# Keep-Passion/ImageStitch

Measured on AMD Instinct MI355X. Metric: image-pairs/sec (2048x2048 grayscale, SURF+BF), higher is better.
Workload: dtype f32

## Files before the change

imagestitch_amd/csrc/surf_kernels.hip:

```cpp
#include "common.h"
#include "detmath.h"
#include <math.h>
#include <float.h>
#include <string.h>
#include <stdlib.h>
#include <algorithm>
#include <vector>

#define GAS __attribute__((address_space(1)))
typedef GAS const uint8_t *g_cu8;
typedef GAS const int32_t *g_ci32;
typedef GAS float *g_f32;
typedef GAS const float *g_cf32;
typedef GAS int32_t *g_i32;
__device__ __forceinline__ int cv_round_f(float v) { return (int)rintf(v); }
__device__ __forceinline__ uint8_t round_u8_pos(float v) { return (uint8_t)__float_as_uint(v + 12582912.f); }
__device__ __forceinline__ int cv_round_d(double v) { return (int)rint(v); }
__device__ __forceinline__ int cv_floor_d(double v) { return (int)floor(v); }
__device__ __forceinline__ int cv_ceil_d(double v) { return (int)ceil(v); }

__device__ __forceinline__ int wave_incl_scan(int v)
{
    const int lane = threadIdx.x & 63;
#pragma unroll
// ... 655 lines not shown
        int t = base + threadIdx.x;
        if (t < n) { SortKey k = make_key(R.cand[t]); t1[threadIdx.x] = k.k1; t2[threadIdx.x] = k.k2; t3[threadIdx.x] = k.k3; }
        __syncthreads();
        const int k0 = part * 64, k1e = min(k0 + 64, n - base);
        if (idx < n) {
            bool tie = false;
#pragma unroll 8
            for (int k = k0; k < k1e; k++) {
                const unsigned long long a = t1[k];
                rank += (a > mk.k1) ? 1 : 0;
                tie |= (a == mk.k1);
            }
            if (tie)
                for (int k = k0; k < k1e; k++)
                    if (t1[k] == mk.k1) rank += (t2[k] < mk.k2 || (t2[k] == mk.k2 && t3[k] < mk.k3)) ? 1 : 0;
        }
        __syncthreads();
    }
    partial[part][lane] = rank;
    __syncthreads();
    if (part == 0 && idx < n) {
        rank = partial[0][lane] + partial[1][lane] + partial[2][lane] + partial[3][lane];
        vfsms_keypoint kp;
        kp.x = me.x; kp.y = me.y; kp.size = me.size; kp.angle = -1.f; kp.response = me.response;
        kp.octave = me.octave; kp.class_id = cand_class_id(R, pats, me);
        R.kps[rank] = kp;
    }
}

#define SORT_BUCKETS 1024
struct SortRec { unsigned long long k1, k2, k3; int idx, pad; };
__device__ __forceinline__ int sort_bucket(unsigned long long k1)
{
    const int b = (int)((uint32_t)(k1 >> 32) >> 18) - (133 << 5);
    return min(max(b, 0), SORT_BUCKETS - 1);
}
__global__ __launch_bounds__(1024) void k_bucket_sort(const RoiDev *rois)
{
    const RoiDev &R = rois[blockIdx.x];
    const int n = min(R.counters[0], R.cap);
    if (n <= 0) return;
    __shared__ int hist[SORT_BUCKETS], base[SORT_BUCKETS], cursor[SORT_BUCKETS], wsum[16];
    const int tid = threadIdx.x, lane = tid & 63, wid = tid >> 6;
    hist[tid] = 0; cursor[tid] = 0;
    __syncthreads();
    for (int i = tid; i < n; i += 1024) atomicAdd(&hist[sort_bucket(make_key(R.cand[i]).k1)], 1);
    __syncthreads();
    {
        const int rb = SORT_BUCKETS - 1 - tid;
        const int v = hist[rb];
        int incl = wave_incl_scan(v);
        if (lane == 63) wsum[wid] = incl;
        __syncthreads();
        int off = 0;
        for (int k = 0; k < wid; k++) off += wsum[k];
        base[rb] = off + incl - v;
    }
    __syncthreads();
    SortRec *S = reinterpret_cast<SortRec *>(R.patch);
    for (int i = tid; i < n; i += 1024) {
        const SortKey k = make_key(R.cand[i]);
        const int b = sort_bucket(k.k1);
        const int pos = base[b] + atomicAdd(&cursor[b], 1);
        SortRec r; r.k1 = k.k1; r.k2 = k.k2; r.k3 = k.k3; r.idx = i; r.pad = 0;
        S[pos] = r;
    }
    R.keep_pos[tid] = base[tid]; R.order[tid] = hist[tid];
}

#define BRANK_STAGE 1024
__global__ __launch_bounds__(256) void k_bucket_rank(const RoiDev *rois, const LayerPat *pats)
{
    const RoiDev &R = rois[blockIdx.y];
    const int n = min(R.counters[0], R.cap);
    const int p0 = blockIdx.x * 256;
    if (p0 >= n) return;
    const int p = p0 + (int)threadIdx.x;
    const bool live = p < n;
    const GAS unsigned long long *S = (const GAS unsigned long long *)R.patch;
    static_assert(sizeof(SortRec) == 32, "k_bucket_rank reads the records as four 64-bit words");
    g_ci32 bpos = (g_ci32)R.keep_pos, bcnt = (g_ci32)R.order;
    __shared__ unsigned long long key1[BRANK_STAGE];
    __shared__ int span[2];
    SortRec me; me.k1 = me.k2 = me.k3 = 0; me.idx = 0;
    int lo = 0, hi = 0;
    if (live) {
        me.k1 = S[4 * p]; me.k2 = S[4 * p + 1]; me.k3 = S[4 * p + 2]; me.idx = (int)(uint32_t)S[4 * p + 3];
        const int b = sort_bucket(me.k1);
        lo = bpos[b]; hi = lo + bcnt[b];
        if (threadIdx.x == 0) span[0] = lo;
        if (p == min(p0 + 255, n - 1)) span[1] = hi;
    }
    __syncthreads();
    const int s0 = span[0], s1 = span[1];
    int rank = lo;
    auto tie = [&](int q) {
        const unsigned long long a2 = S[4 * q + 1], a3 = S[4 * q + 2];
        return (a2 < me.k2 || (a2 == me.k2 && a3 < me.k3)) ? 1 : 0;
    };
    if (s1 - s0 <= BRANK_STAGE) {
        for (int q = s0 + (int)threadIdx.x; q < s1; q += 256) key1[q - s0] = S[4 * q];
        __syncthreads();
        if (live) {
            int q = lo;
            for (; q + 4 <= hi; q += 4) {
                unsigned long long a[4];
#pragma unroll
                for (int u = 0; u < 4; u++) a[u] = key1[q - s0 + u];
#pragma unroll
                for (int u = 0; u < 4; u++) {
                    rank += (a[u] > me.k1) ? 1 : 0;
                    if (a[u] == me.k1 && q + u != p) rank += tie(q + u);
                }
            }
            for (; q < hi; q++) {
                const unsigned long long a1 = key1[q - s0];
                rank += (a1 > me.k1) ? 1 : 0;
                if (a1 == me.k1 && q != p) rank += tie(q);
            }
        }
    } else if (live) {
        for (int q = lo; q < hi; q++) {
            const unsigned long long a1 = S[4 * q];
            rank += (a1 > me.k1) ? 1 : 0;
            if (a1 == me.k1 && q != p) rank += tie(q);
        }
    }
    if (!live) return;
    Cand c;
    {
        constexpr int CW = sizeof(Cand) / 4;
        g_ci32 src = (g_ci32)R.cand + (size_t)me.idx * CW;
        int32_t *cw = (int32_t *)&c;
#pragma unroll
        for (int w = 0; w < CW; w++) cw[w] = src[w];
    }
    vfsms_keypoint kp;
    kp.x = c.x; kp.y = c.y; kp.size = c.size; kp.angle = -1.f; kp.response = c.response;
    kp.octave = c.octave; kp.class_id = cand_class_id(R, pats, c);
    {
        constexpr int KW = sizeof(vfsms_keypoint) / 4;
        g_i32 dst = (g_i32)R.kps + (size_t)rank * KW;
        const int32_t *kw = (const int32_t *)&kp;
#pragma unroll
        for (int w = 0; w < KW; w++) dst[w] = kw[w];
    }
}

__device__ __forceinline__ float fast_atan2_deg(float y, float x)
{
    const float s = (float)(180 / 3.1415926535897932384626433832795);
    const float p1 = 0.9997878412794807f * s, p3 = -0.3258083974640975f * s;
    const float p5 = 0.1555786518463281f * s, p7 = -0.04432655554792128f * s;
    float ax = fabsf(x), ay = fabsf(y);
    float a, c, c2;
    if (ax >= ay) {
        c = ay / (ax + (float)DBL_EPSILON);
        c2 = c * c;
        a = (((p7 * c2 + p5) * c2 + p3) * c2 + p1) * c;
    } else {
        c = ax / (ay + (float)DBL_EPSILON);
        c2 = c * c;
        a = 90.f - (((p7 * c2 + p5) * c2 + p3) * c2 + p1) * c;
    }
    if (x < 0) a = 180.f - a;
    if (y < 0) a = 360.f - a;
    return a;
}

#ifndef ORI_KP
#define ORI_KP 2
#endif
typedef float ori_f2 __attribute__((ext_vector_type(2)));
__device__ __forceinline__ void orientation_block(const RoiDev &R, const SurfTables *T, const int k0, const int n, int upright)
{
    __shared__ __attribute__((aligned(16))) float2 XY[ORI_KP][128];
    __shared__ __attribute__((aligned(16))) uint8_t Zb[ORI_KP][9][128];
    __shared__ float mod_s[ORI_KP][72], sx_s[ORI_KP][72], sy_s[ORI_KP][72];
    __shared__ int nvalid[ORI_KP], state[ORI_KP];
    const int tid = threadIdx.x;
    const int kq = __builtin_amdgcn_readfirstlane(tid >> 7), t = tid & 127;
    if (tid < ORI_KP) { nvalid[tid] = 0; state[tid] = 0; }
    __syncthreads();
    {
        const int k = k0 + kq;
        int valid = 0;
        uint32_t m0 = 0, m1 = 0, m2 = 0;
        float2 xy = make_float2(0.f, 0.f);
        if (k < n) {
            const vfsms_keypoint kp = R.kps[k];
            const float s = kp.size * 1.2f / 9.0f;
            const int gws = 2 * cv_round_f(2 * s);
            const int srows = R.h + 1, scols = R.w + 1, sw = R.w + 1;
            if (srows < gws || scols < gws) {
                if (t == 0) { R.kps[k].size = -1.f; state[kq] = 1; }
            } else if (upright) {
                if (t == 0) { R.kps[k].angle = 270.f; state[kq] = 1; }
            } else if (t < T->nOriSamples) {
                int x = cv_round_f(kp.x + T->aptx[t] * s - (float)(gws - 1) / 2);
                int y = cv_round_f(kp.y + T->apty[t] * s - (float)(gws - 1) / 2);
                if (!(y < 0 || y >= srows - gws || x < 0 || x >= scols - gws)) {
                    const float ratio = (float)gws / 4;
                    const int r2 = cv_round_f(ratio * 2), r4 = cv_round_f(ratio * 4);
                    g_ci32 p0 = (g_ci32)R.sum + (size_t)y * sw + x;
                    g_ci32 p2 = p0 + (size_t)r2 * sw, p4 = p0 + (size_t)r4 * sw;
                    const int a00 = p0[0], a02 = p0[r2], a04 = p0[r4];
                    const int a20 = p2[0], a24 = p2[r4];
                    const int a40 = p4[0], a42 = p4[r2], a44 = p4[r4];
                    const float wA = 1.f / ((float)r2 * (float)r4);
                    float wB = wA;
                    if (r4 - r2 != r2) wB = 1.f / ((float)(r4 - r2) * (float)r4);
                    const int vx0 = a00 + a42 - a40 - a02, vx1 = a02 + a44 - a42 - a04;
                    const int vy0 = a00 + a24 - a20 - a04, vy1 = a20 + a44 - a40 - a24;
                    double dxd = 0; dxd += (double)(-((float)vx0 * wA)); dxd += (double)((float)vx1 * wB);
                    double dyd = 0; dyd += (double)((float)vy0 * wA); dyd += (double)(-((float)vy1 * wB));
                    const float vx = (float)dxd, vy = (float)dyd;
                    const float aw = T->aptw[t];
                    const float xx = vx * aw, yy = vy * aw;
                    xy = make_float2(xx, yy);
                    const int ang = cv_round_f(fast_atan2_deg(yy, xx));
                    const uint32_t *mrow = T->oriMask[min(max(ang, 0), 360)];
                    m0 = mrow[0]; m1 = mrow[1]; m2 = mrow[2];
                    valid = 1;
                }
            }
        } else if (t == 0) state[kq] = 1;
        XY[kq][t] = xy;
        Zb[kq][0][t] = (uint8_t)m0; Zb[kq][1][t] = (uint8_t)(m0 >> 8); Zb[kq][2][t] = (uint8_t)(m0 >> 16); Zb[kq][3][t] = (uint8_t)(m0 >> 24);
        Zb[kq][4][t] = (uint8_t)m1; Zb[kq][5][t] = (uint8_t)(m1 >> 8); Zb[kq][6][t] = (uint8_t)(m1 >> 16); Zb[kq][7][t] = (uint8_t)(m1 >> 24);
        Zb[kq][8][t] = (uint8_t)m2;
        const unsigned long long m = __ballot(valid);
        if ((tid & 63) == 0 && m) atomicAdd(&nvalid[kq], __popcll(m));
    }
    __syncthreads();
    if (tid < ORI_KP * 72) {
        const int q = tid / 72, w = tid - q * 72;
        if (state[q] == 0 && nvalid[q] > 0) {
            const int nori = T->nOriSamples;
            const uint8_t *zrow = Zb[q][w >> 3];
            const int bit = w & 7;
            ori_f2 acc = {0.f, 0.f};
            for (int j = 0; j < nori; j += 8) {
                const uint2 z8 = *reinterpret_cast<const uint2 *>(&zrow[j]);
                const uint32_t za = (z8.x >> bit) & 0x01010101u, zb = (z8.y >> bit) & 0x01010101u;
                const float4 p01 = *reinterpret_cast<const float4 *>(&XY[q][j]), p23 = *reinterpret_cast<const float4 *>(&XY[q][j + 2]);
                const float4 p45 = *reinterpret_cast<const float4 *>(&XY[q][j + 4]), p67 = *reinterpret_cast<const float4 *>(&XY[q][j + 6]);
#define ORI_ACC(Z, N, P, XC, YC) do { float mf; asm("v_cvt_f32_ubyte" #N " %0, %1" : "=v"(mf) : "v"(Z)); \
                                           acc = __builtin_elementwise_fma((ori_f2){P.XC, P.YC}, (ori_f2){mf, mf}, acc); } while (0)
                ORI_ACC(za, 0, p01, x, y); ORI_ACC(za, 1, p01, z, w); ORI_ACC(za, 2, p23, x, y); ORI_ACC(za, 3, p23, z, w);
                ORI_ACC(zb, 0, p45, x, y); ORI_ACC(zb, 1, p45, z, w); ORI_ACC(zb, 2, p67, x, y); ORI_ACC(zb, 3, p67, z, w);
#undef ORI_ACC
            }
            const float sumx = acc.x, sumy = acc.y;
            mod_s[q][w] = sumx * sumx + sumy * sumy;
            sx_s[q][w] = sumx; sy_s[q][w] = sumy;
        }
    }
    __syncthreads();
    {
        const int q = __builtin_amdgcn_readfirstlane(tid >> 6), lane = tid & 63;
        if (q < ORI_KP && state[q] == 0) {
            const int k = k0 + q;
            if (nvalid[q] == 0) {
                if (lane == 0) R.kps[k].size = -1.f;
            } else {
                float bm = mod_s[q][lane]; int bi = lane;
                if (!(bm > 0.f)) bm = 0.f;
                if (lane < 8) { float m2 = mod_s[q][64 + lane]; if (m2 > bm) { bm = m2; bi = 64 + lane; } }
#pragma unroll
                for (int off = 32; off >= 1; off >>= 1) {
                    const float om = __shfl_xor(bm, off, 64); const int oi = __shfl_xor(bi, off, 64);
                    if (om > bm || (om == bm && oi < bi)) { bm = om; bi = oi; }
                }
                if (lane == 0) {
                    float bestx = 0, besty = 0;
                    if (bm > 0.f) { bestx = sx_s[q][bi]; besty = sy_s[q][bi]; }
                    R.kps[k].angle = fast_atan2_deg(-besty, bestx);
                }
            }
        }
    }
}

#ifdef VFSMS_DESC_TIMING
__device__ unsigned long long g_desc_cycles[8];
#define DT_MARK(ph) do { if (threadIdx.x == 0) { unsigned long long _n = clock64(); atomicAdd(&g_desc_cycles[ph], _n - _t0); _t0 = _n; } } while (0)
#define DT_START unsigned long long _t0 = clock64()
extern "C" int vfsms_debug_desc_cycles(unsigned long long *out) { return hipMemcpyFromSymbol(out, HIP_SYMBOL(g_desc_cycles), sizeof(unsigned long long) * 8) == hipSuccess ? 0 : -3; }
__device__ unsigned long long g_desc_trips[4];
#define DT_TRIP(n) do {} while (0)
__device__ unsigned long long g_desc_unit_cycles[4];
#define DT_UNIT_BEGIN unsigned long long _u0 = clock64()
#define DT_UNIT_END(n) do { _uacc[n] += clock64() - _u0; _ucnt[n]++; } while (0)
extern "C" int vfsms_debug_desc_unit_cycles(unsigned long long *out) { return hipMemcpyFromSymbol(out, HIP_SYMBOL(g_desc_unit_cycles), sizeof(unsigned long long) * 4) == hipSuccess ? 0 : -3; }
extern "C" int vfsms_debug_desc_trips(unsigned long long *out) { return hipMemcpyFromSymbol(out, HIP_SYMBOL(g_desc_trips), sizeof(unsigned long long) * 4) == hipSuccess ? 0 : -3; }
#else
#define DT_MARK(ph) do {} while (0)
#define DT_START do {} while (0)
#define DT_TRIP(n) do {} while (0)
#define DT_UNIT_BEGIN do {} while (0)
#define DT_UNIT_END(n) do {} while (0)
#endif
#ifndef VFSMS_EXP
#define VFSMS_EXP 0
#endif
#ifndef DESC_WBUF
#define DESC_WBUF 15360
#endif
__device__ __forceinline__ void origin_chain(float *row, float s, const float d, const int n)
{
    int i = 0;
    for (; i + 4 <= n; i += 4) {
        const float a = s, b = a + d, c = b + d, e = c + d;
        s = e + d;
        row[i] = a; row[i + 1] = b; row[i + 2] = c; row[i + 3] = e;
    }
    for (; i < n; i++, s += d) row[i] = s;
}

struct WinGeom {
    int win; float sin_dir, cos_dir;
    int h, w, stride; g_cu8 img;
    g_cu8 pair;
    int upright, usx, usy;
};

__device__ __forceinline__ int win_sample_xy(const WinGeom &G, double px, double py)
{
    const int ncols1 = G.w - 1, nrows1 = G.h - 1;
    const int ix = (int)px, iy = (int)py;
    if (px >= 0.0 && py >= 0.0 && ix < ncols1 && iy < nrows1) {
        const float a = (float)__builtin_amdgcn_fract(px), b = (float)__builtin_amdgcn_fract(py);
        g_cu8 p = G.img + (size_t)iy * G.stride + ix;
        const float v = p[0] * (1.f - a) * (1.f - b) + p[1] * a * (1.f - b) + p[G.stride] * (1.f - a) * b + p[G.stride + 1] * a * b;
        return (int)(uint8_t)cv_round_f(v);
    }
    const int x = min(max(cv_round_d(px), 0), ncols1);
    const int y = min(max(cv_round_d(py), 0), nrows1);
    return (int)G.img[(size_t)y * G.stride + x];
}
__device__ __forceinline__ int win_sample_upright(const WinGeom &G, int i, int j)
{
    const int x = min(max(G.usx + i, 0), G.w - 1);
    const int y = min(max(G.usy - j, 0), G.h - 1);
    return (int)G.img[(size_t)y * G.stride + x];
}

typedef float float2v __attribute__((ext_vector_type(2)));
__device__ __forceinline__ float bilinear_pk(uint32_t top, float a, float b)
{
    const float na = 1.f - a, nb = 1.f - b;
    const float2v w = {na, a};
    const float2v r0 = {(float)(top & 0xff), (float)((top >> 16) & 0xff)};
    const float2v r1 = {(float)((top >> 8) & 0xff), (float)(top >> 24)};
    float2v p = r0 * w, q = r1 * w;
    const float2v nb2 = {nb, nb}, b2 = {b, b};
    p = p * nb2; q = q * b2;
    return ((p.x + p.y) + q.x) + q.y;
}
#ifndef STAGE_ILP
#define STAGE_ILP 4
#endif
#define UNIT_W (8 * STAGE_ILP)
#ifndef BORDER_ILP
#define BORDER_ILP 2
#endif
#ifndef STAGE_FRAC_FIRST
#define STAGE_FRAC_FIRST 1
#endif
template <int N>
__device__ __forceinline__ void stage_round(g_cu8 ubase, const uint32_t pw, const double c, const double sn, const double sxc, const double syc,
                                            const int jlane, uint8_t *wrow)
{
    uint32_t top[N];
    const double jd = (double)jlane;
    const double px0 = __builtin_fma(jd, c, sxc), py0 = __builtin_fma(jd, -sn, syc);
#if STAGE_FRAC_FIRST
    float fa[N], fb[N];
#pragma unroll
    for (int u = 0; u < N; u++) {
        const double px = u ? px0 + (double)(8 * u) * c : px0, py = u ? py0 - (double)(8 * u) * sn : py0;
        const uint32_t off = ((uint32_t)__umul24((uint32_t)(int)py, pw) + (uint32_t)(int)px) << 1;
        fa[u] = (float)__builtin_amdgcn_fract(px); fb[u] = (float)__builtin_amdgcn_fract(py);
        top[u] = *(GAS const uint32_t *)(ubase + off);
    }
#pragma unroll
    for (int u = 0; u < N; u++) wrow[8 * u] = round_u8_pos(bilinear_pk(top[u], fa[u], fb[u]));
#else
    double px[N], py[N];
    px[0] = px0; py[0] = py0;
#pragma unroll
    for (int u = 1; u < N; u++) { px[u] = px[0] + (double)(8 * u) * c; py[u] = py[0] - (double)(8 * u) * sn; }
#pragma unroll
    for (int u = 0; u < N; u++) {
        const uint32_t off = ((uint32_t)__umul24((uint32_t)(int)py[u], pw) + (uint32_t)(int)px[u]) << 1;
        top[u] = *(GAS const uint32_t *)(ubase + off);
    }
#pragma unroll
    for (int u = 0; u < N; u++) {
        const float a = (float)__builtin_amdgcn_fract(px[u]), b = (float)__builtin_amdgcn_fract(py[u]);
        wrow[8 * u] = round_u8_pos(bilinear_pk(top[u], a, b));
    }
#endif
}

template <int NW>
__device__ __forceinline__ void stage_rows(const WinGeom &G, const float *sx_row, const float *sy_row,
                                           int r0, int nrows, uint8_t *dst, uint8_t *strip_in)
{
    const int win = __builtin_amdgcn_readfirstlane(G.win);
    r0 = __builtin_amdgcn_readfirstlane(r0); nrows = __builtin_amdgcn_readfirstlane(nrows);
    const int lane = threadIdx.x & 63, wv = NW == 1 ? 0 : __builtin_amdgcn_readfirstlane((int)(threadIdx.x >> 6));
    const int li = lane >> 3, lj = lane & 7;
    const int strips = (nrows + 7) >> 3;
    const double c = (double)G.cos_dir, sn = (double)G.sin_dir;
    const int ncols1 = __builtin_amdgcn_readfirstlane(G.w) - 1, nrows1 = __builtin_amdgcn_readfirstlane(G.h) - 1;
    const uint64_t bp = (uint64_t)G.pair;
    g_cu8 ubase = (g_cu8)(((uint64_t)(uint32_t)__builtin_amdgcn_readfirstlane((uint32_t)(bp >> 32)) << 32) |
                          (uint64_t)(uint32_t)__builtin_amdgcn_readfirstlane((uint32_t)bp));
    const uint32_t pw = (uint32_t)(ncols1 + 1);
    const int gfull = win >> 3, tailc = win & 7;
    int nb = NW == 1 ? 1 : (gfull + 7) >> 3;
#if VFSMS_EXP & 16
    nb = (gfull + 3) >> 2;
#endif
    const int gbase = gfull / nb, grem = gfull - gbase * nb;
    const int total = strips * nb;
    if (!G.upright) {
        const int tid = NW == 1 ? lane : (int)threadIdx.x;
        if (tid < strips) {
            const int ia = min(r0 + tid * 8, VFSMS_MAX_WIN - 1), ib = min(min(r0 + tid * 8 + 7, r0 + nrows - 1), VFSMS_MAX_WIN - 1);
// ... 233 lines not shown
            __syncthreads();
            DT_MARK(3);
            for (int p0 = 0; p0 < cn; p0 += DESC_PASS) {
                const int pn = min(DESC_PASS, cn - p0);
                for (int e = threadIdx.x; e < pn * 21; e += 256) {
                    const int r = (int)(((uint32_t)e * 3121u) >> 16), dx = e - 21 * r;
                    if (tail_ok) {
                        const AreaRec cx = REC[dx];
                        float w[AREA_TAIL];
                        area_tail_weights(cx, nmin, w);
                        rowsum[e] = area_row_tab_w(WINBUF + (p0 + r) * win, cx, nmin, nmax, w);
                    } else
                        rowsum[e] = area_row_tab(WINBUF + (p0 + r) * win, REC[dx], nmin, nmax);
                }
                __syncthreads();
                const int s0 = c0 + p0, s1 = s0 + pn;
                for (int o = threadIdx.x; o < 441; o += 256) {
                    const int dy = (int)(((uint32_t)o * 3121u) >> 16), dx = o - 21 * dy;
                    const AreaRec ry = REC[dy];
                    const int a = max(ry.j0, s0), b = min(ry.j0 + ry.n, s1);
                    if (dy < dyA || dy >= dyB || a >= b) continue;
                    float sum = a == ry.j0 ? 0.f : acc[o];
                    for (int s = a; s < b; s++) {
                        const int t = s - ry.j0;
                        const float rb = rowsum[(s - s0) * 21 + dx];
                        if (t == 0) sum = ry.a0 * rb;
                        else sum += (t < ry.n - 1 ? ry.af : ry.al) * rb;
                    }
                    if (b == ry.j0 + ry.n) PATCH[dy][dx] = area_out(sum, mode, inv_area);
                    else acc[o] = sum;
                }
                if (p0 + DESC_PASS < cn) __syncthreads();
            }
            DT_MARK(4);
        }
    }
    __syncthreads();
    if (band >= 0) {
        if (threadIdx.x < 21) R.patch[(size_t)k * VFSMS_PATCH_ROW + band * 21 + threadIdx.x] = PATCH[band][threadIdx.x];
    } else {
        for (int o = threadIdx.x; o < 441; o += 256) R.patch[(size_t)k * VFSMS_PATCH_ROW + o] = PATCH[o / 21][o % 21];
    }
    DT_MARK(5);
}

#define DESC_NCLS 4

__device__ __forceinline__ int desc_class(float size)
{
    const float s = size * 1.2f / 9.0f;
    const int win = min((int)((20 + 1) * s), VFSMS_MAX_WIN);
    return win > 256 ? 0 : win > 128 ? 1 : win > 64 ? 2 : 3;
}

__global__ __launch_bounds__(1024) void k_desc_order(const RoiDev *rois)
{
    const RoiDev &R = rois[blockIdx.x];
    const int n = min(R.counters[0], R.cap);
    __shared__ int cnt[DESC_NCLS], base[DESC_NCLS], cur[DESC_NCLS];
    if (threadIdx.x < DESC_NCLS) { cnt[threadIdx.x] = 0; cur[threadIdx.x] = 0; }
    __syncthreads();
    const int lane = threadIdx.x & 63;
    for (int k0 = 0; k0 < n; k0 += 1024) {
        const int k = k0 + threadIdx.x;
        const float size = k < n ? R.kps[k].size : -1.f;
        const int cls = size > 0 ? desc_class(size) : -1;
#pragma unroll
        for (int c = 0; c < DESC_NCLS; c++) {
            const unsigned long long m = __ballot(cls == c);
            if (m && lane == __ffsll((long long)m) - 1) atomicAdd(&cnt[c], __popcll(m));
        }
    }
    __syncthreads();
    if (threadIdx.x == 0) {
        int acc = 0;
        for (int c = 0; c < DESC_NCLS; c++) { base[c] = acc; acc += cnt[c]; R.counters[12 + c] = cnt[c]; }
    }
    __syncthreads();
    for (int k0 = 0; k0 < n; k0 += 1024) {
        const int k = k0 + threadIdx.x;
        const float size = k < n ? R.kps[k].size : -1.f;
        const int cls = size > 0 ? desc_class(size) : -1;
#pragma unroll
        for (int c = 0; c < DESC_NCLS; c++) {
            const unsigned long long m = __ballot(cls == c);
            if (!m) continue;
            const int leader = __ffsll((long long)m) - 1;
            int start = 0;
            if (lane == leader) start = atomicAdd(&cur[c], __popcll(m));
            start = __shfl(start, leader, 64);
            if (cls == c) R.order[base[c] + start + __popcll(m & ((1ull << lane) - 1))] = k;
        }
    }
}

#define DESC_HEADS DESC_PLAN_HEADS
#define DESC_HEAD_STRIDE 64

__global__ __launch_bounds__(256) void k_desc_plan(const RoiDev *rois, int nrois, DescPlan *plan, int big_grid)
{
    __shared__ int c[VFSMS_MAX_ROIS][4];
    for (int e = threadIdx.x; e < nrois * 4; e += 256) c[e >> 2][e & 3] = rois[e >> 2].counters[12 + (e & 3)];
    __syncthreads();
    if (threadIdx.x == 0) {
        int acc = 0, total = 0;
        for (int q = 0; q < DESC_HEADS; q++) {
            plan->big_start[q] = acc;
            for (int r = q; r < nrois; r += DESC_HEADS) { plan->seg_base[r][0] = acc; acc += c[r][0]; }
            plan->big_n0[q] = acc - plan->big_start[q];
            for (int r = q; r < nrois; r += DESC_HEADS) {
                plan->seg_base[r][1] = acc; acc += c[r][1];
                plan->seg_base[r][2] = acc; acc += c[r][2];
            }
            plan->big_tickets[q] = acc - plan->big_start[q];
        }
        total = acc;
        const int split = total < big_grid * 48 ? 21 : 1;
        plan->split = split;
        for (int q = 0; q < DESC_HEADS; q++) plan->big_tickets[q] += (split - 1) * plan->big_n0[q];
        acc = 0;
        for (int q = 0; q < DESC_HEADS; q++) {
            plan->small_start[q] = acc;
            for (int r = q; r < nrois; r += DESC_HEADS) { plan->seg_base[r][3] = acc; acc += c[r][3]; }
            plan->small_tickets[q] = acc - plan->small_start[q];
        }
    }
}

__global__ __launch_bounds__(256) void k_desc_recs(const RoiDev *rois, const DescPlan *plan, DescRec *big, DescRec *small, int upright)
{
    const int roi = blockIdx.y;
    const RoiDev &R = rois[roi];
    const int p = blockIdx.x * 256 + threadIdx.x;
    const int c0 = R.counters[12], c1 = R.counters[13], c2 = R.counters[14], c3 = R.counters[15];
    if (p >= c0 + c1 + c2 + c3) return;
    const int cls = p < c0 ? 0 : p < c0 + c1 ? 1 : p < c0 + c1 + c2 ? 2 : 3;
    const int idx = p - (cls > 0 ? c0 : 0) - (cls > 1 ? c1 : 0) - (cls > 2 ? c2 : 0);
    const int k = R.order[p];
    const vfsms_keypoint kp = R.kps[k];
    DescRec rec;
    rec.roi = roi; rec.k = k; rec.pad = 0; rec.x = kp.x; rec.y = kp.y;
    rec.win = (int)((20 + 1) * (kp.size * 1.2f / 9.0f));
    rec.sin_dir = 0.f; rec.cos_dir = 0.f;
    if (!upright) {
        const float dir = kp.angle * (float)(3.1415926535897932384626433832795 / 180);
        double sd, cd;
        det_sincos((double)dir, &sd, &cd);
        rec.sin_dir = -(float)sd;
        rec.cos_dir = (float)cd;
    }
    (cls < 3 ? big : small)[plan->seg_base[roi][cls] + idx] = rec;
}

__global__ __launch_bounds__(ORI_KP * 128, 8) void k_orientation(const RoiDev *rois, const SurfTables *T, int upright)
{
    const RoiDev &R = rois[blockIdx.y];
    const int n = min(R.counters[0], R.cap);
    const int k0 = blockIdx.x * ORI_KP;
    if (k0 >= n) return;
    orientation_block(R, T, k0, n, upright);
}

#define DESC_SMALL_WIN 64
struct SmallLds { uint8_t win[DESC_SMALL_WIN * DESC_SMALL_WIN + 64]; float sx[DESC_SMALL_WIN + 8], sy[DESC_SMALL_WIN + 8]; AreaRec rec[AREA_RECS]; int rec_win; uint8_t strip_in[DESC_SMALL_WIN / 8 + 8]; };

__device__ __forceinline__ void wave_sync_lds()
{
    __builtin_amdgcn_fence(__ATOMIC_ACQ_REL, "wavefront");
    __builtin_amdgcn_wave_barrier();
}

__device__ void describe_small(const RoiDev &R, const AreaRec *area_tab, const DescRec &rec, int upright, SmallLds &L)
{
    const int lane = threadIdx.x & 63;
    const int k = rec.k;
    WinGeom G;
    G.win = min(rec.win, DESC_SMALL_WIN);
    G.h = R.h; G.w = R.w; G.stride = R.stride; G.img = (g_cu8)R.img; G.pair = (g_cu8)R.pair;
    G.upright = upright; G.usx = 0; G.usy = 0; G.sin_dir = rec.sin_dir; G.cos_dir = rec.cos_dir;
    const int win = G.win;
    const int dsz = 21;
    if (L.rec_win != win) {
        wave_sync_lds();
        const int *src = (const int *)(area_tab + (size_t)max(win, dsz) * AREA_RECS);
        for (int e = lane; e < AREA_RECS * 8; e += 64) ((int *)L.rec)[e] = src[e];
        if (lane == 0) L.rec_win = win;
    }
    if (!upright) {
        const float sin_dir = rec.sin_dir, cos_dir = rec.cos_dir;
        if (lane < 2) {
            const float win_offset = -(float)(win - 1) / 2;
            const float sx0 = rec.x + win_offset * cos_dir + win_offset * sin_dir, sy0 = rec.y - win_offset * sin_dir + win_offset * cos_dir;
            origin_chain(lane == 0 ? L.sx : L.sy, lane == 0 ? sx0 : sy0, lane == 0 ? sin_dir : cos_dir, win);
        }
    } else {
        const float win_offset = -(float)(win - 1) / 2;
        G.usx = cv_round_f(rec.x + win_offset);
        G.usy = cv_round_f(rec.y - win_offset);
    }
    wave_sync_lds();
    stage_rows<1>(G, L.sx, L.sy, 0, win, L.win, L.strip_in);
    wave_sync_lds();
    const int nmin = __builtin_amdgcn_readfirstlane(L.rec[21].j0), nmax = __builtin_amdgcn_readfirstlane(L.rec[21].n);
    const int mode = __builtin_amdgcn_readfirstlane(L.rec[21].mode);
    const float inv_area = L.rec[21].a0;
    const bool tail_ok = nmax - max(nmin - 1, 1) <= AREA_TAIL;
    uint8_t *prow = R.patch + (size_t)k * VFSMS_PATCH_ROW;
    for (int o = lane; o < dsz * dsz; o += 64) {
        const int dy = (int)(((uint32_t)o * 3121u) >> 16), dx = o - dsz * dy;
        const AreaRec ry = L.rec[dy], rx = L.rec[dx];
        const uint8_t *S = L.win + ry.j0 * win;
        float sum;
        if (tail_ok) {
            float w[AREA_TAIL];
            area_tail_weights(rx, nmin, w);
            sum = ry.a0 * area_row_tab_w(S, rx, nmin, nmax, w);
            for (int ty = 1; ty < nmax; ty++) {
                const float beta = ty < ry.n - 1 ? ry.af : (ty == ry.n - 1 ? ry.al : 0.f);
                sum += beta * area_row_tab_w(S + ty * win, rx, nmin, nmax, w);
            }
        } else {
            sum = ry.a0 * area_row_tab(S, rx, nmin, nmax);
            for (int ty = 1; ty < nmax; ty++) {
                const float beta = ty < ry.n - 1 ? ry.af : (ty == ry.n - 1 ? ry.al : 0.f);
                sum += beta * area_row_tab(S + ty * win, rx, nmin, nmax);
            }
        }
        uint8_t outv;
        if (mode == 2) outv = (uint8_t)(((int)sum + 2) >> 2);
        else if (mode == 1) outv = sat_u8(sum * inv_area);
        else outv = sat_u8(sum);
        prow[o] = outv;
    }
    wave_sync_lds();
}

#ifndef DESC_SMALL_WGS
#define DESC_SMALL_WGS 7
#endif
__device__ __forceinline__ DescRec load_rec_uniform(const DescRec *p)
{
    const int *q = (const int *)p;
    DescRec r;
    r.roi = __builtin_amdgcn_readfirstlane(q[0]); r.k = __builtin_amdgcn_readfirstlane(q[1]);
    r.win = __builtin_amdgcn_readfirstlane(q[2]); r.pad = 0;
    r.sin_dir = __int_as_float(__builtin_amdgcn_readfirstlane(q[4])); r.cos_dir = __int_as_float(__builtin_amdgcn_readfirstlane(q[5]));
    r.x = __int_as_float(__builtin_amdgcn_readfirstlane(q[6])); r.y = __int_as_float(__builtin_amdgcn_readfirstlane(q[7]));
    return r;
}
__global__ __launch_bounds__(256, DESC_SMALL_WGS) void k_describe_small(const RoiDev *rois, const DescPlan *plan, const DescRec *recs, int *counter,
                                                                 const AreaRec *area_tab, int upright)
{
    __shared__ SmallLds L[4];
    if (threadIdx.x < 4) L[threadIdx.x].rec_win = -1;
    __syncthreads();
    const int lane = threadIdx.x & 63, wave = __builtin_amdgcn_readfirstlane((int)(threadIdx.x >> 6));
    int head = 0;
    for (;;) {
        int slot = -1;
        if (lane == 0)
            while (head < DESC_HEADS) {
                const int q = (blockIdx.x + head) & (DESC_HEADS - 1);
                const int n = plan->small_tickets[q];
                const int t = n > 0 ? atomicAdd(counter + q * DESC_HEAD_STRIDE, 1) : 0;
                if (t < n) { slot = plan->small_start[q] + t; break; }
                head++;
            }
        slot = __builtin_amdgcn_readfirstlane(slot);
        head = __builtin_amdgcn_readfirstlane(head);
        if (slot < 0) break;
        const DescRec rec = load_rec_uniform(recs + slot);
        describe_small(rois[rec.roi], area_tab, rec, upright, L[wave]);
    }
}

__global__ __launch_bounds__(256) void k_pair_rows(const RoiDev *rois)
{
    const RoiDev &R = rois[blockIdx.z];
    const int y = blockIdx.y, x = (blockIdx.x * 256 + threadIdx.x) * 4;
    if (y >= R.h || x >= R.w) return;
    g_cu8 r0 = (g_cu8)R.img + (size_t)y * R.stride + x, r1 = (g_cu8)R.img + (size_t)min(y + 1, R.h - 1) * R.stride + x;
    GAS uint16_t *dst = (GAS uint16_t *)R.pair + (size_t)y * R.w + x;
    if (x + 4 <= R.w) {
        const uint32_t a = *(GAS const u32u *)r0, b = *(GAS const u32u *)r1;
#pragma unroll
        for (int k = 0; k < 4; k++) dst[k] = (uint16_t)(((a >> (8 * k)) & 0xff) | (((b >> (8 * k)) & 0xff) << 8));
    } else {
        for (int k = 0; x + k < R.w; k++) dst[k] = (uint16_t)(r0[k] | (r1[k] << 8));
    }
}

#ifndef DESC_WGS
#define DESC_WGS 6
#endif
__global__ __launch_bounds__(256, DESC_WGS) void k_describe(const RoiDev *rois, const DescPlan *plan, const DescRec *recs, int *counter, const SurfTables *T,
                                                  const AreaRec *area_tab, int extended, int upright)
{
    __shared__ int s_slot, s_band;
    int head = 0;
#ifdef VFSMS_DESC_TIMING
    unsigned long long tq = clock64();
#endif
    for (;;) {
        __syncthreads();
        if (threadIdx.x == 0) {
            int slot = -1, band = -1;
            const int split = plan->split;
            while (head < DESC_HEADS) {
                const int q = (blockIdx.x + head) & (DESC_HEADS - 1);
                const int n = plan->big_tickets[q];
                const int t = n > 0 ? atomicAdd(counter + q * DESC_HEAD_STRIDE, 1) : 0;
                if (t < n) {
                    const int n0 = plan->big_n0[q];
                    if (t < n0 * split) { slot = plan->big_start[q] + t / split; band = split > 1 ? t % split : -1; }
                    else slot = plan->big_start[q] + n0 + (t - n0 * split);
                    break;
                }
                head++;
            }
            s_slot = slot; s_band = band;
        }
        __syncthreads();
        const int slot = __builtin_amdgcn_readfirstlane(s_slot), band = __builtin_amdgcn_readfirstlane(s_band);
// ... 133 lines not shown
    d->tickets = a.take<int>(2 * DESC_HEADS * DESC_HEAD_STRIDE);
    d->plan = a.take<DescPlan>(1);
    d->rec_big = a.take<DescRec>(capsum);
    d->rec_small = a.take<DescRec>(capsum);
}

int launch_surf_detect(vfsms_ctx *ctx, const RoiDev *d_rois, const RoiDev *h_rois, int nrois,
                       const vfsms_surf_params *p)
{
    if (nrois <= 0) return VFSMS_OK;
    const int lpo = p->n_octave_layers + 2;
    int maxcap = 0;
    for (int r = 0; r < nrois; r++) maxcap = h_rois[r].cap > maxcap ? h_rois[r].cap : maxcap;
    const std::vector<ShapeRun> runs = shape_runs(h_rois, nrois);
    {
        ProfScope ps(ctx, "integral");
        for (const ShapeRun &q : runs) TRY(launch_integral(ctx, d_rois + q.first, q.count, q.h, q.w));
    }
    {
        ProfScope ps(ctx, "hessian");
        static const bool generic = getenv("VFSMS_HESSIAN_GENERIC") && atoi(getenv("VFSMS_HESSIAN_GENERIC")) != 0;
        for (const ShapeRun &q : runs) {
            const RoiDev *dq = d_rois + q.first;
            int step = 1, o = 0;
            if (lpo == 5) {
                for (; o < p->n_octaves && o < 2; o++) {
                    const int lrows = q.h / step, lcols = q.w / step;
                    if (lrows > 0 && lcols > 0) {
                        if (o == 0)
                            hipLaunchKernelGGL((k_hessian_lds<1, 64, 4>), dim3((lcols + 63) / 64, (lrows + 15) / 16, q.count), dim3(64, 4), 0, ctx->stream, dq, ctx->d_layers.as<LayerPat>(), lpo, o);
                        else
                            hipLaunchKernelGGL((k_hessian_lds<2, 32, HESS_O1_WAVES>), dim3((lcols + 31) / 32, (lrows + 15) / 16, q.count), dim3(64, HESS_O1_WAVES), 0, ctx->stream, dq, ctx->d_layers.as<LayerPat>(), lpo, o);
                    }
                    step *= 2;
                }
            }
            static const bool rows2 = !(getenv("VFSMS_HESSIAN_ROWS2") && atoi(getenv("VFSMS_HESSIAN_ROWS2")) == 0);
            if (lpo == 5 && o == 2 && o < p->n_octaves && rows2 && !generic) {
                const int s0 = 36;
                if (q.h >= s0 && q.w >= s0) {
                    const int tiles_i = ((q.h - s0) / 4 + 1 + 1) / 2, tiles_j = ((q.w - s0) / 4 + 1 + 127) / 128;
                    hipLaunchKernelGGL(k_hessian_rows2, dim3((unsigned)(tiles_i * tiles_j * 5 * q.count)), dim3(64, 4), 0, ctx->stream, dq, ctx->d_layers.as<LayerPat>(), lpo,
                                       tiles_i, tiles_j, q.count);
                }
                o++; step *= 2;
            }
            HessPlan plan; plan.o0 = o; plan.noct = 0; plan.first[0] = 0;
            for (; o < p->n_octaves && plan.noct < VFSMS_MAX_OCTAVES; o++) {
                const int lrows = q.h / step, lcols = q.w / step;
                const int tx = (lcols + 63) / 64, ty = (lrows + 3) / 4;
                plan.tiles_x[plan.noct] = tx > 0 ? tx : 1;
                plan.first[plan.noct + 1] = plan.first[plan.noct] + tx * ty;
                plan.noct++;
                step *= 2;
            }
            if (plan.noct > 0 && plan.first[plan.noct] > 0) {
                if (lpo == 5 && plan.o0 >= 2 && plan.o0 + plan.noct <= 4 && !generic)
                    hipLaunchKernelGGL(k_hessian_coarse, dim3((unsigned)plan.first[plan.noct] * lpo * q.count), dim3(64, 4), 0, ctx->stream, dq, ctx->d_layers.as<LayerPat>(), lpo, plan, q.count);
                else
                    hipLaunchKernelGGL(k_hessian, dim3((unsigned)plan.first[plan.noct] * lpo * q.count), dim3(64, 4), 0, ctx->stream, dq, ctx->d_layers.as<LayerPat>(), lpo, plan, q.count);
            }
        }
    }
    {
        ProfScope ps(ctx, "nms");
        for (const ShapeRun &q : runs) {
            NmsPlan plan; plan.noct = 0; plan.first[0] = 0;
            int step = 1;
            for (int o = 0; o < p->n_octaves && o < VFSMS_MAX_OCTAVES; o++) {
                const int lrows = q.h / step, lcols = q.w / step;
                const int tx = (lcols + NMS_TW - 1) / NMS_TW, ty = (lrows + NMS_TH - 1) / NMS_TH;
                plan.tiles_x[o] = tx > 0 ? tx : 1;
                plan.first[o + 1] = plan.first[o] + tx * ty;
                plan.noct = o + 1;
                step *= 2;
            }
            if (plan.noct > 0 && plan.first[plan.noct] > 0)
                hipLaunchKernelGGL(k_nms, dim3(plan.first[plan.noct], q.count * p->n_octave_layers), dim3(64, 4), 0, ctx->stream, d_rois + q.first,
                                   ctx->d_layers.as<LayerPat>(), lpo, p->n_octave_layers, plan, p->hessian_threshold);
        }
    }
    {
        ProfScope ps(ctx, "sort");
        static const bool n2sort = getenv("VFSMS_SORT_N2") && atoi(getenv("VFSMS_SORT_N2")) != 0;
        int mincap = maxcap;
        for (int r = 0; r < nrois; r++) mincap = h_rois[r].cap < mincap ? h_rois[r].cap : mincap;
        if (n2sort || mincap < SORT_BUCKETS) hipLaunchKernelGGL(k_rank_sort, dim3((maxcap + 63) / 64, nrois), dim3(256), 0, ctx->stream, d_rois, ctx->d_layers.as<LayerPat>());
        else {
            hipLaunchKernelGGL(k_bucket_sort, dim3(nrois), dim3(1024), 0, ctx->stream, d_rois);
            hipLaunchKernelGGL(k_bucket_rank, dim3((maxcap + 255) / 256, nrois), dim3(256), 0, ctx->stream, d_rois, ctx->d_layers.as<LayerPat>());
        }
    }
    HIP_TRY(hipGetLastError());
    return VFSMS_OK;
}


int ctx_prepare_area_tab(vfsms_ctx *ctx)
{
    if (ctx->d_area_tab) return VFSMS_OK;
    std::vector<AreaRec> tab((size_t)(VFSMS_MAX_WIN + 1) * AREA_RECS);
    memset(tab.data(), 0, sizeof(AreaRec) * tab.size());
    const int dsz = 21;
    for (int win = dsz; win <= VFSMS_MAX_WIN; win++) {
        AreaRec *rec = tab.data() + (size_t)win * AREA_RECS;
        const double inv_scale = (double)dsz / win;
        const double scale = 1. / inv_scale;
        const int iscale = (int)rint(scale);
        const bool fast = fabs(scale - iscale) < DBL_EPSILON;
        int nmin = 1 << 30, nmax = 0;
        for (int dx = 0; dx < dsz; dx++) {
            AreaRec &c = rec[dx];
            if (fast) { c.j0 = dx * iscale; c.n = iscale; c.a0 = c.af = c.al = 1.f; }
            else {
                const double fsx1 = dx * scale;
                const double fsx2 = fsx1 + scale;
                const double cellWidth = fmin(scale, win - fsx1);
                int sx1 = (int)ceil(fsx1), sx2 = (int)floor(fsx2);
                sx2 = std::min(sx2, win - 1);
                sx1 = std::min(sx1, sx2);
                const bool left = sx1 - fsx1 > 1e-3, right = fsx2 - sx2 > 1e-3;
                const float a_left = (float)((sx1 - fsx1) / cellWidth), a_full = (float)(1.0 / cellWidth);
                const float a_right = (float)(fmin(fmin(fsx2 - sx2, 1.), cellWidth) / cellWidth);
                c.j0 = left ? sx1 - 1 : sx1;
                c.n = (left ? 1 : 0) + (sx2 - sx1) + (right ? 1 : 0);
                c.a0 = left ? a_left : (sx2 > sx1 ? a_full : a_right);
                c.af = a_full;
                c.al = right ? a_right : a_full;
                if (c.n == 1 && left) c.al = a_left;
            }
            if (c.n < 1 || c.j0 < 0 || c.j0 + c.n > win) { vfsms_set_error("internal: INTER_AREA table of window %d", win); return VFSMS_ERR_UNSUPPORTED; }
            nmin = std::min(nmin, c.n); nmax = std::max(nmax, c.n);
        }
        if (nmax > 40) { vfsms_set_error("internal: INTER_AREA run of window %d", win); return VFSMS_ERR_UNSUPPORTED; }
        rec[21].j0 = nmin; rec[21].n = nmax; rec[21].a0 = fast ? 1.f / (iscale * iscale) : 1.f;
        rec[21].mode = !fast ? 0 : iscale == 2 ? 2 : 1;
    }
    for (int win = 0; win < dsz; win++) memcpy(tab.data() + (size_t)win * AREA_RECS, tab.data() + (size_t)dsz * AREA_RECS, sizeof(AreaRec) * AREA_RECS);
    TRY(ctx->d_area_tab.reserve(sizeof(AreaRec) * tab.size(), ctx->stream));
    HIP_TRY(hipMemcpy(ctx->d_area_tab.as<void>(), tab.data(), sizeof(AreaRec) * tab.size(), hipMemcpyHostToDevice));
    return VFSMS_OK;
}

int launch_surf_describe(vfsms_ctx *ctx, const RoiDev *d_rois, const RoiDev *h_rois, int nrois,
                         const vfsms_surf_params *p)
{
    if (nrois <= 0) return VFSMS_OK;
    if (nrois > VFSMS_MAX_ROIS) { vfsms_set_error("more than %d ROIs in one batch", VFSMS_MAX_ROIS); return VFSMS_ERR_CAPACITY; }
    TRY(ctx_prepare_area_tab(ctx));
    int maxcap = 0;
    for (int r = 0; r < nrois; r++) maxcap = h_rois[r].cap > maxcap ? h_rois[r].cap : maxcap;
    {
        ProfScope ps(ctx, "orientation");
        hipLaunchKernelGGL(k_orientation, dim3((maxcap + ORI_KP - 1) / ORI_KP, nrois), dim3(ORI_KP * 128), 0, ctx->stream, d_rois, ctx->d_tables.as<SurfTables>(), p->upright);
    }
    {
        ProfScope ps(ctx, "compact");
        hipLaunchKernelGGL(k_keep_scan, dim3(nrois), dim3(1024), 0, ctx->stream, d_rois);
    }
    {
        ProfScope ps(ctx, "describe");
        size_t capsum = 0;
        for (int r = 0; r < nrois; r++) capsum += (size_t)h_rois[r].cap;
        ArenaWalk a = ctx_arena_walk(ctx); DescWork W;
        surf_describe_layout(a, &W, capsum);
        TRY(ctx_arena_commit(ctx, a, "arena exhausted (descriptor work list)"));
        HIP_TRY(hipMemsetAsync(W.tickets, 0, sizeof(int) * 2 * DESC_HEADS * DESC_HEAD_STRIDE, ctx->stream));
        for (const ShapeRun &q : shape_runs(h_rois, nrois))
            hipLaunchKernelGGL(k_pair_rows, dim3((q.w + 1023) / 1024, q.h, q.count), dim3(256), 0, ctx->stream, d_rois + q.first);
        hipLaunchKernelGGL(k_desc_order, dim3(nrois), dim3(1024), 0, ctx->stream, d_rois);
        hipLaunchKernelGGL(k_desc_plan, dim3(1), dim3(256), 0, ctx->stream, d_rois, nrois, W.plan, 256 * DESC_WGS);
        hipLaunchKernelGGL(k_desc_recs, dim3((maxcap + 255) / 256, nrois), dim3(256), 0, ctx->stream, d_rois, W.plan, W.rec_big, W.rec_small, p->upright);
        hipLaunchKernelGGL(k_describe, dim3(256 * DESC_WGS), dim3(256), 0, ctx->stream, d_rois, W.plan, W.rec_big, W.tickets,
                           ctx->d_tables.as<SurfTables>(), ctx->d_area_tab.as<AreaRec>(), p->extended, p->upright);
        hipLaunchKernelGGL(k_describe_small, dim3(256 * DESC_SMALL_WGS), dim3(256), 0, ctx->stream, d_rois, W.plan, W.rec_small,
                           W.tickets + DESC_HEADS * DESC_HEAD_STRIDE, ctx->d_area_tab.as<AreaRec>(), p->upright);
        hipLaunchKernelGGL(k_desc_tail, dim3((maxcap + 15) / 16, nrois), dim3(256), 0, ctx->stream, d_rois, ctx->d_tables.as<SurfTables>(), p->extended);
    }
    HIP_TRY(hipGetLastError());
    return VFSMS_OK;
}
```

Baseline: 2514.

## Map one wavefront per keypoint in SURF orientation kernel

New measurement: 2602 (median of 6 runs). +3.5%, better.

```diff
diff --git a/imagestitch_amd/csrc/surf_kernels.hip b/imagestitch_amd/csrc/surf_kernels.hip
--- a/imagestitch_amd/csrc/surf_kernels.hip
+++ b/imagestitch_amd/csrc/surf_kernels.hip
@@ -831,131 +831,169 @@
     const float s = (float)(180 / 3.1415926535897932384626433832795);
     const float p1 = 0.9997878412794807f * s, p3 = -0.3258083974640975f * s;
     const float p5 = 0.1555786518463281f * s, p7 = -0.04432655554792128f * s;
-    float ax = fabsf(x), ay = fabsf(y);
-    float a, c, c2;
-    if (ax >= ay) {
-        c = ay / (ax + (float)DBL_EPSILON);
-        c2 = c * c;
-        a = (((p7 * c2 + p5) * c2 + p3) * c2 + p1) * c;
-    } else {
-        c = ax / (ay + (float)DBL_EPSILON);
-        c2 = c * c;
-        a = 90.f - (((p7 * c2 + p5) * c2 + p3) * c2 + p1) * c;
-    }
+    const float ax = fabsf(x), ay = fabsf(y);
+    const bool xge = ax >= ay;
+    const float num = xge ? ay : ax, den = (xge ? ax : ay) + (float)DBL_EPSILON;
+    const float c = num / den;
+    const float c2 = c * c;
+    float a = (((p7 * c2 + p5) * c2 + p3) * c2 + p1) * c;
+    a = xge ? a : 90.f - a;
     if (x < 0) a = 180.f - a;
     if (y < 0) a = 360.f - a;
     return a;
 }
 
-#ifndef ORI_KP
-#define ORI_KP 2
+__device__ __forceinline__ void wave_sync_lds()
+{
+    __builtin_amdgcn_fence(__ATOMIC_ACQ_REL, "wavefront");
+    __builtin_amdgcn_wave_barrier();
+}
+
+#ifndef ORI_K
+#define ORI_K 4
 #endif
+#define ORI_XY_ROW 130
+#define ORI_Z_ROW 136
 typedef float ori_f2 __attribute__((ext_vector_type(2)));
+
+struct OriTaps { int a00, a02, a04, a20, a24, a40, a42, a44; };
+
+__device__ __forceinline__ bool ori_taps(const RoiDev &R, const SurfTables *T, int nori, float kx, float ky, float s, int gws, int r2, int r4, int t, OriTaps &a)
+{
+    const int srows = R.h + 1, scols = R.w + 1, sw = R.w + 1;
+    const int tc = max(min(t, nori - 1), 0);
+    const int x = cv_round_f(kx + T->aptx[tc] * s - (float)(gws - 1) / 2);
+    const int y = cv_round_f(ky + T->apty[tc] * s - (float)(gws - 1) / 2);
+    const bool in = t < nori && !(y < 0 || y >= srows - gws || x < 0 || x >= scols - gws);
+    const int e2 = in ? r2 : 0, e4 = in ? r4 : 0;
+    g_ci32 p0 = (g_ci32)R.sum + (in ? (size_t)y * sw + x : (size_t)0);
+    g_ci32 p2 = p0 + (size_t)e2 * sw, p4 = p0 + (size_t)e4 * sw;
+    a.a00 = p0[0]; a.a02 = p0[e2]; a.a04 = p0[e4];
+    a.a20 = p2[0]; a.a24 = p2[e4];
+    a.a40 = p4[0]; a.a42 = p4[e2]; a.a44 = p4[e4];
+    return in;
+}
+
+struct OriSample { float xx, yy; uint32_t m0, m1, m2; };
+
+__device__ __forceinline__ OriSample ori_gradient(const SurfTables *T, int nori, const OriTaps &a, float wA, float wB, int t)
+{
+    const int vx0 = a.a00 + a.a42 - a.a40 - a.a02, vx1 = a.a02 + a.a44 - a.a42 - a.a04;
+    const int vy0 = a.a00 + a.a24 - a.a20 - a.a04, vy1 = a.a20 + a.a44 - a.a40 - a.a24;
+    double dxd = 0; dxd += (double)(-((float)vx0 * wA)); dxd += (double)((float)vx1 * wB);
+    double dyd = 0; dyd += (double)((float)vy0 * wA); dyd += (double)(-((float)vy1 * wB));
+    const float vx = (float)dxd, vy = (float)dyd;
+    const float aw = T->aptw[max(min(t, nori - 1), 0)];
+    const float xx = vx * aw, yy = vy * aw;
+    const int ang = cv_round_f(fast_atan2_deg(yy, xx));
+    const uint32_t *mrow = T->oriMask[min(max(ang, 0), 360)];
+    OriSample o;
+    o.xx = xx; o.yy = yy; o.m0 = mrow[0]; o.m1 = mrow[1]; o.m2 = mrow[2];
+    return o;
+}
+
+__device__ __forceinline__ void ori_store(bool in, const OriSample &o, int t, float2 *xyq, uint8_t *zq)
+{
+    const uint32_t m0 = in ? o.m0 : 0u, m1 = in ? o.m1 : 0u, m2 = in ? o.m2 : 0u;
+    xyq[t] = make_float2(in ? o.xx : 0.f, in ? o.yy : 0.f);
+    zq[0 * ORI_Z_ROW + t] = (uint8_t)m0; zq[1 * ORI_Z_ROW + t] = (uint8_t)(m0 >> 8); zq[2 * ORI_Z_ROW + t] = (uint8_t)(m0 >> 16); zq[3 * ORI_Z_ROW + t] = (uint8_t)(m0 >> 24);
+    zq[4 * ORI_Z_ROW + t] = (uint8_t)m1; zq[5 * ORI_Z_ROW + t] = (uint8_t)(m1 >> 8); zq[6 * ORI_Z_ROW + t] = (uint8_t)(m1 >> 16); zq[7 * ORI_Z_ROW + t] = (uint8_t)(m1 >> 24);
+    zq[8 * ORI_Z_ROW + t] = (uint8_t)m2;
+}
+
+__device__ __forceinline__ ori_f2 ori_window_sum(const float2 *xyq, const uint8_t *zq, int w, int nori)
+{
+    const uint8_t *zrow = zq + (w >> 3) * ORI_Z_ROW;
+    const int bit = w & 7;
+    ori_f2 acc = {0.f, 0.f};
+    for (int j = 0; j < nori; j += 8) {
+        const uint2 z8 = *reinterpret_cast<const uint2 *>(&zrow[j]);
+        const uint32_t za = (z8.x >> bit) & 0x01010101u, zb = (z8.y >> bit) & 0x01010101u;
+        const float4 p01 = *reinterpret_cast<const float4 *>(&xyq[j]), p23 = *reinterpret_cast<const float4 *>(&xyq[j + 2]);
+        const float4 p45 = *reinterpret_cast<const float4 *>(&xyq[j + 4]), p67 = *reinterpret_cast<const float4 *>(&xyq[j + 6]);
+#define ORI_ACC(Z, N, P, XC, YC) do { float mf; asm("v_cvt_f32_ubyte" #N " %0, %1" : "=v"(mf) : "v"(Z)); \
+                                   acc = __builtin_elementwise_fma((ori_f2){P.XC, P.YC}, (ori_f2){mf, mf}, acc); } while (0)
+        ORI_ACC(za, 0, p01, x, y); ORI_ACC(za, 1, p01, z, w); ORI_ACC(za, 2, p23, x, y); ORI_ACC(za, 3, p23, z, w);
+        ORI_ACC(zb, 0, p45, x, y); ORI_ACC(zb, 1, p45, z, w); ORI_ACC(zb, 2, p67, x, y); ORI_ACC(zb, 3, p67, z, w);
+#undef ORI_ACC
+    }
+    return acc;
+}
+
 __device__ __forceinline__ void orientation_block(const RoiDev &R, const SurfTables *T, const int k0, const int n, int upright)
 {
-    __shared__ __attribute__((aligned(16))) float2 XY[ORI_KP][128];
-    __shared__ __attribute__((aligned(16))) uint8_t Zb[ORI_KP][9][128];
-    __shared__ float mod_s[ORI_KP][72], sx_s[ORI_KP][72], sy_s[ORI_KP][72];
-    __shared__ int nvalid[ORI_KP], state[ORI_KP];
-    const int tid = threadIdx.x;
-    const int kq = __builtin_amdgcn_readfirstlane(tid >> 7), t = tid & 127;
-    if (tid < ORI_KP) { nvalid[tid] = 0; state[tid] = 0; }
-    __syncthreads();
-    {
-        const int k = k0 + kq;
-        int valid = 0;
-        uint32_t m0 = 0, m1 = 0, m2 = 0;
-        float2 xy = make_float2(0.f, 0.f);
-        if (k < n) {
-            const vfsms_keypoint kp = R.kps[k];
-            const float s = kp.size * 1.2f / 9.0f;
-            const int gws = 2 * cv_round_f(2 * s);
-            const int srows = R.h + 1, scols = R.w + 1, sw = R.w + 1;
-            if (srows < gws || scols < gws) {
-                if (t == 0) { R.kps[k].size = -1.f; state[kq] = 1; }
-            } else if (upright) {
-                if (t == 0) { R.kps[k].angle = 270.f; state[kq] = 1; }
-            } else if (t < T->nOriSamples) {
-                int x = cv_round_f(kp.x + T->aptx[t] * s - (float)(gws - 1) / 2);
-                int y = cv_round_f(kp.y + T->apty[t] * s - (float)(gws - 1) / 2);
-                if (!(y < 0 || y >= srows - gws || x < 0 || x >= scols - gws)) {
-                    const float ratio = (float)gws / 4;
-                    const int r2 = cv_round_f(ratio * 2), r4 = cv_round_f(ratio * 4);
-                    g_ci32 p0 = (g_ci32)R.sum + (size_t)y * sw + x;
-                    g_ci32 p2 = p0 + (size_t)r2 * sw, p4 = p0 + (size_t)r4 * sw;
-                    const int a00 = p0[0], a02 = p0[r2], a04 = p0[r4];
-                    const int a20 = p2[0], a24 = p2[r4];
-                    const int a40 = p4[0], a42 = p4[r2], a44 = p4[r4];
-                    const float wA = 1.f / ((float)r2 * (float)r4);
-                    float wB = wA;
-                    if (r4 - r2 != r2) wB = 1.f / ((float)(r4 - r2) * (float)r4);
-                    const int vx0 = a00 + a42 - a40 - a02, vx1 = a02 + a44 - a42 - a04;
-                    const int vy0 = a00 + a24 - a20 - a04, vy1 = a20 + a44 - a40 - a24;
-                    double dxd = 0; dxd += (double)(-((float)vx0 * wA)); dxd += (double)((float)vx1 * wB);
-                    double dyd = 0; dyd += (double)((float)vy0 * wA); dyd += (double)(-((float)vy1 * wB));
-                    const float vx = (float)dxd, vy = (float)dyd;
-                    const float aw = T->aptw[t];
-                    const float xx = vx * aw, yy = vy * aw;
-                    xy = make_float2(xx, yy);
-                    const int ang = cv_round_f(fast_atan2_deg(yy, xx));
-                    const uint32_t *mrow = T->oriMask[min(max(ang, 0), 360)];
-                    m0 = mrow[0]; m1 = mrow[1]; m2 = mrow[2];
-                    valid = 1;
-                }
-            }
-        } else if (t == 0) state[kq] = 1;
-        XY[kq][t] = xy;
-        Zb[kq][0][t] = (uint8_t)m0; Zb[kq][1][t] = (uint8_t)(m0 >> 8); Zb[kq][2][t] = (uint8_t)(m0 >> 16); Zb[kq][3][t] = (uint8_t)(m0 >> 24);
-        Zb[kq][4][t] = (uint8_t)m1; Zb[kq][5][t] = (uint8_t)(m1 >> 8); Zb[kq][6][t] = (uint8_t)(m1 >> 16); Zb[kq][7][t] = (uint8_t)(m1 >> 24);
-        Zb[kq][8][t] = (uint8_t)m2;
-        const unsigned long long m = __ballot(valid);
-        if ((tid & 63) == 0 && m) atomicAdd(&nvalid[kq], __popcll(m));
-    }
-    __syncthreads();
-    if (tid < ORI_KP * 72) {
-        const int q = tid / 72, w = tid - q * 72;
-        if (state[q] == 0 && nvalid[q] > 0) {
-            const int nori = T->nOriSamples;
-            const uint8_t *zrow = Zb[q][w >> 3];
-            const int bit = w & 7;
-            ori_f2 acc = {0.f, 0.f};
-            for (int j = 0; j < nori; j += 8) {
-                const uint2 z8 = *reinterpret_cast<const uint2 *>(&zrow[j]);
-                const uint32_t za = (z8.x >> bit) & 0x01010101u, zb = (z8.y >> bit) & 0x01010101u;
-                const float4 p01 = *reinterpret_cast<const float4 *>(&XY[q][j]), p23 = *reinterpret_cast<const float4 *>(&XY[q][j + 2]);
-                const float4 p45 = *reinterpret_cast<const float4 *>(&XY[q][j + 4]), p67 = *reinterpret_cast<const float4 *>(&XY[q][j + 6]);
-#define ORI_ACC(Z, N, P, XC, YC) do { float mf; asm("v_cvt_f32_ubyte" #N " %0, %1" : "=v"(mf) : "v"(Z)); \
-                                           acc = __builtin_elementwise_fma((ori_f2){P.XC, P.YC}, (ori_f2){mf, mf}, acc); } while (0)
-                ORI_ACC(za, 0, p01, x, y); ORI_ACC(za, 1, p01, z, w); ORI_ACC(za, 2, p23, x, y); ORI_ACC(za, 3, p23, z, w);
-                ORI_ACC(zb, 0, p45, x, y); ORI_ACC(zb, 1, p45, z, w); ORI_ACC(zb, 2, p67, x, y); ORI_ACC(zb, 3, p67, z, w);
-#undef ORI_ACC
-            }
-            const float sumx = acc.x, sumy = acc.y;
-            mod_s[q][w] = sumx * sumx + sumy * sumy;
-            sx_s[q][w] = sumx; sy_s[q][w] = sumy;
-        }
-    }
-    __syncthreads();
-    {
-        const int q = __builtin_amdgcn_readfirstlane(tid >> 6), lane = tid & 63;
-        if (q < ORI_KP && state[q] == 0) {
-            const int k = k0 + q;
-            if (nvalid[q] == 0) {
-                if (lane == 0) R.kps[k].size = -1.f;
-            } else {
-                float bm = mod_s[q][lane]; int bi = lane;
-                if (!(bm > 0.f)) bm = 0.f;
-                if (lane < 8) { float m2 = mod_s[q][64 + lane]; if (m2 > bm) { bm = m2; bi = 64 + lane; } }
-#pragma unroll
-                for (int off = 32; off >= 1; off >>= 1) {
-                    const float om = __shfl_xor(bm, off, 64); const int oi = __shfl_xor(bi, off, 64);
-                    if (om > bm || (om == bm && oi < bi)) { bm = om; bi = oi; }
-                }
-                if (lane == 0) {
-                    float bestx = 0, besty = 0;
-                    if (bm > 0.f) { bestx = sx_s[q][bi]; besty = sy_s[q][bi]; }
-                    R.kps[k].angle = fast_atan2_deg(-besty, bestx);
-                }
+    __shared__ __attribute__((aligned(16))) float2 XY[ORI_K][ORI_XY_ROW];
+    __shared__ __attribute__((aligned(16))) uint8_t Zb[ORI_K][9 * ORI_Z_ROW];
+    __shared__ float mod_l[ORI_K][8], sx_l[ORI_K][8], sy_l[ORI_K][8];
+    __shared__ int live[ORI_K];
+    const int tid = threadIdx.x, lane = tid & 63;
+    const int q = __builtin_amdgcn_readfirstlane(tid >> 6);
+    const int k = k0 + q;
+    int compute = 0, nvalid = 0;
+    const int nori = T->nOriSamples;
+    if (k < n) {
+        typedef const float __attribute__((address_space(4))) *ori_cf32;
+        const float kx = *(ori_cf32)(uintptr_t)&R.kps[k].x, ky = *(ori_cf32)(uintptr_t)&R.kps[k].y;
+        const float ksize = *(ori_cf32)(uintptr_t)&R.kps[k].size;
+        const float s = ksize * 1.2f / 9.0f;
+        const int gws = 2 * cv_round_f(2 * s);
+        if (R.h + 1 < gws || R.w + 1 < gws) {
+            if (lane == 0) R.kps[k].size = -1.f;
+        } else if (upright) {
+            if (lane == 0) R.kps[k].angle = 270.f;
+        } else {
+            compute = 1;
+            const float ratio = (float)gws / 4;
+            const int r2 = cv_round_f(ratio * 2), r4 = cv_round_f(ratio * 4);
+            const float wA = 1.f / ((float)r2 * (float)r4);
+            float wB = wA;
+            if (r4 - r2 != r2) wB = 1.f / ((float)(r4 - r2) * (float)r4);
+            OriTaps a0, a1;
+            const bool in0 = ori_taps(R, T, nori, kx, ky, s, gws, r2, r4, lane, a0);
+            const bool in1 = ori_taps(R, T, nori, kx, ky, s, gws, r2, r4, 64 + lane, a1);
+            nvalid = __popcll(__ballot(in0)) + __popcll(__ballot(in1));
+            if (nvalid > 0) {
+                const OriSample o0 = ori_gradient(T, nori, a0, wA, wB, lane), o1 = ori_gradient(T, nori, a1, wA, wB, 64 + lane);
+                ori_store(in0, o0, lane, XY[q], Zb[q]);
+                ori_store(in1, o1, 64 + lane, XY[q], Zb[q]);
+            }
+        }
+    }
+    const int sums = compute && nvalid > 0;
+    if (lane == 0) live[q] = sums;
+    ori_f2 own = {0.f, 0.f};
+    if (sums) {
+        wave_sync_lds();
+        own = ori_window_sum(XY[q], Zb[q], lane, nori);
+    }
+    __syncthreads();
+    if (q == 0 && lane < ORI_K * 8) {
+        const int lq = lane >> 3, lw = lane & 7;
+        if (live[lq]) {
+            const ori_f2 acc = ori_window_sum(XY[lq], Zb[lq], 64 + lw, nori);
+            mod_l[lq][lw] = acc.x * acc.x + acc.y * acc.y;
+            sx_l[lq][lw] = acc.x; sy_l[lq][lw] = acc.y;
+        }
+    }
+    __syncthreads();
+    if (compute) {
+        if (nvalid == 0) {
+            if (lane == 0) R.kps[k].size = -1.f;
+        } else {
+            float bm = own.x * own.x + own.y * own.y; int bi = lane;
+            if (!(bm > 0.f)) bm = 0.f;
+            if (lane < 8) { float m2 = mod_l[q][lane]; if (m2 > bm) { bm = m2; bi = 64 + lane; } }
+#pragma unroll
+            for (int off = 32; off >= 1; off >>= 1) {
+                const float om = __shfl_xor(bm, off, 64); const int oi = __shfl_xor(bi, off, 64);
+                const bool take = (om > bm) | ((om == bm) & (oi < bi));
+                bm = take ? om : bm; bi = take ? oi : bi;
+            }
+            const float ownx = __shfl(own.x, bi & 63, 64), owny = __shfl(own.y, bi & 63, 64);
+            if (lane == 0) {
+                float bestx = 0, besty = 0;
+                if (bm > 0.f) { bestx = bi < 64 ? ownx : sx_l[q][bi - 64]; besty = bi < 64 ? owny : sy_l[q][bi - 64]; }
+                R.kps[k].angle = fast_atan2_deg(-besty, bestx);
             }
         }
     }
@@ -1495,23 +1533,17 @@
     (cls < 3 ? big : small)[plan->seg_base[roi][cls] + idx] = rec;
 }
 
-__global__ __launch_bounds__(ORI_KP * 128, 8) void k_orientation(const RoiDev *rois, const SurfTables *T, int upright)
+__global__ __launch_bounds__(ORI_K * 64, 8) void k_orientation(const RoiDev *rois, const SurfTables *T, int upright)
 {
     const RoiDev &R = rois[blockIdx.y];
-    const int n = min(R.counters[0], R.cap);
-    const int k0 = blockIdx.x * ORI_KP;
+    const int n = min(*(const int __attribute__((address_space(4))) *)(uintptr_t)R.counters, R.cap);
+    const int k0 = blockIdx.x * ORI_K;
     if (k0 >= n) return;
     orientation_block(R, T, k0, n, upright);
 }
 
 #define DESC_SMALL_WIN 64
 struct SmallLds { uint8_t win[DESC_SMALL_WIN * DESC_SMALL_WIN + 64]; float sx[DESC_SMALL_WIN + 8], sy[DESC_SMALL_WIN + 8]; AreaRec rec[AREA_RECS]; int rec_win; uint8_t strip_in[DESC_SMALL_WIN / 8 + 8]; };
-
-__device__ __forceinline__ void wave_sync_lds()
-{
-    __builtin_amdgcn_fence(__ATOMIC_ACQ_REL, "wavefront");
-    __builtin_amdgcn_wave_barrier();
-}
 
 __device__ void describe_small(const RoiDev &R, const AreaRec *area_tab, const DescRec &rec, int upright, SmallLds &L)
 {
@@ -1951,7 +1983,7 @@
     for (int r = 0; r < nrois; r++) maxcap = h_rois[r].cap > maxcap ? h_rois[r].cap : maxcap;
     {
         ProfScope ps(ctx, "orientation");
-        hipLaunchKernelGGL(k_orientation, dim3((maxcap + ORI_KP - 1) / ORI_KP, nrois), dim3(ORI_KP * 128), 0, ctx->stream, d_rois, ctx->d_tables.as<SurfTables>(), p->upright);
+        hipLaunchKernelGGL(k_orientation, dim3((maxcap + ORI_K - 1) / ORI_K, nrois), dim3(ORI_K * 64), 0, ctx->stream, d_rois, ctx->d_tables.as<SurfTables>(), p->upright);
     }
     {
         ProfScope ps(ctx, "compact");
```
